# AIGC-Audio/AudioGPT

Hardware: NVIDIA H100
Metric: mel_frames_per_s_vocoded (higher is better)
Workload: dtype f32

## Files before the change

### audiogpt_b200/csrc/tcconv5.cu

```cuda
#include "tapconv.cuh"
#include "tapconv_epi.cuh"
#include "tc_common.cuh"
#include "tc_h16.cuh"
#include "tc_tma.cuh"
#include "models.h"

#include <set>

namespace agpt {

namespace {

constexpr int MAX_NA = 4, MAX_NW = 8;
constexpr int kMaxDyn = 227 * 1024 - 256;
constexpr int kDualDyn = 113 * 1024 - 256;

struct Tc5Smem {
  uint32_t a_hi[MAX_NA], a_lo[MAX_NA], w[MAX_NW], raw[2], rowinfo, rowp, bars, total;
};
__host__ __device__ inline void tc5_layout(Tc5Smem& s, int BN, int MT, int RRA, int NA, int NW, int NR, bool pl = false,
                                           int raw_pitch = 256) {
  uint32_t o = 0;
  for (int i = 0; i < MAX_NA; ++i) { s.a_hi[i] = o; if (i < NA) o += RRA * 128; }
  for (int i = 0; i < MAX_NA; ++i) { s.a_lo[i] = o; if (i < NA) o += RRA * 128; }
// ... 455 lines not shown
        const int a = rowinfo[row];
        const bool ok = (a >= 0) && (ch < P1.Cin);
        const int slot = ((u >> 1) + ((u & 1) << 2)) ^ (((row >> 2) & 1) << 2);
        cp_async16_zfill(dst + row * 128 + (slot << 4), ok ? (ing + a + ch) : P1.in, ok ? 16u : 0u);
      }
      cp_async_commit_();
    };
    if constexpr (HALF) {
      issue_half(0, 0);
      if (NR == 2) issue_half(1, 1);
    } else {
      issue_raw1(0, 0);
      if (NR == 2 && nchunks > 1) issue_raw1(1, 1);
    }
    {
      const int lines = (BN * 4) / 128 > 0 ? (BN * 4) / 128 : 1;
      for (int idx = xt; idx < MT * lines; idx += NWK) {
        const int p = rowp[idx / lines];
        const int co = (idx % lines) * 32;
        if (p >= 0 && co < P2.Cout) {
          asm volatile("prefetch.global.L2 [%0];" ::"l"(P2.res + g * P2.res_gstride + (long)p * P2.res_pitch + co));
          if (P2.epi == EPI_ACC && P2.accumulate)
            asm volatile("prefetch.global.L2 [%0];" ::"l"(P2.out + g * P2.out_gstride + (long)p * P2.out_pitch + co));
        }
      }
    }
    float acc[MB][NJ][NB / 2];
    zero_tile(acc);
    int it = 0, prev = -1;
    auto mma_taps = [&](const TapConvParams& Q, uint32_t ahi0, uint32_t alo0, int ksteps) {
      for (int t = 0; t < Q.ntaps; ++t, ++it) {
        const int s = it % NW;
        mbar_wait(&w_full[s], (uint32_t)((it / NW) & 1));
        const uint32_t shift = (uint32_t)Q.tap_off[t] * 128u;
        mma_group(acc, make_desc(ahi0 + shift), make_desc(alo0 + shift), smem_u32(smem + S.w[s]), ksteps, w_empty, prev);
        prev = s;
      }
    };
    for (int c = 0; c < nchunks; ++c) {
      const int buf = c % NA;
      const int rb = (NR == 2) ? (c & 1) : 0;
      const int kv = min(H_KCH, P1.Cin - c * H_KCH);
      const int nq = ((kv + 15) >> 4) << 1;
      if constexpr (!HALF) {
        if (NR == 2 && c + 1 < nchunks) asm volatile("cp.async.wait_group 1;" ::: "memory");
        else cp_async_wait_all_();
        named_bar_sync(1, NWK);
      }
      uint8_t* ahi = smem + S.a_hi[buf];
      uint8_t* alo = smem + S.a_lo[buf];
      if constexpr (HALF) {
      const int nh = (kv + 31) >> 5;
      for (int h = 0; h < nh; ++h) {
        if (NR == 2 && h + 1 < nh) asm volatile("cp.async.wait_group 1;" ::: "memory");
        else cp_async_wait_all_();
        named_bar_sync(1, NWK);
        const uint8_t* rawb = smem + S.raw[NR == 2 ? h : 0];
#pragma unroll 2
        for (int idx = xt; idx < RRA * 4; idx += NWK) {
          const int row = ((idx >> 5) << 3) + ((idx >> 3) & 3) + (((idx >> 2) & 1) << 2), q = idx & 3, qg = 4 * h + q;
          if (qg >= nq) continue;
          const int sw = ((row >> 2) & 1) << 6;
          const float4 x0 = pro_apply5(P1, *reinterpret_cast<const float4*>(rawb + row * 128 + ((q * 16) ^ sw)), true, nullptr);
          const float4 x1 = pro_apply5(P1, *reinterpret_cast<const float4*>(rawb + row * 128 + ((64 + q * 16) ^ sw)), true, nullptr);
          uint4 hv, lv;
          split8(x0, x1, hv, lv);
          const uint32_t o = sw128(row, qg);
          *reinterpret_cast<uint4*>(ahi + o) = hv;
          *reinterpret_cast<uint4*>(alo + o) = lv;
        }
        if (NR == 1 && h + 1 < nh) {
          named_bar_sync(1, NWK);
          issue_half(h + 1, 0);
        }
      }
      fence_proxy_async();
      named_bar_sync(1, NWK);
      } else {
      const uint8_t* rawb = smem + S.raw[rb];
#pragma unroll 2
      for (int idx = xt; idx < RRA * 8; idx += NWK) {
        const int row = idx >> 3, q = idx & 7;
        if (q >= nq) continue;
        const float4 x0 = pro_apply5(P1, *reinterpret_cast<const float4*>(rawb + row * 256 + q * 16), true, nullptr);
        const float4 x1 = pro_apply5(P1, *reinterpret_cast<const float4*>(rawb + row * 256 + 128 + q * 16), true, nullptr);
        uint4 h, l;
        split8(x0, x1, h, l);
        const uint32_t o = sw128(row, q);
        *reinterpret_cast<uint4*>(ahi + o) = h;
        *reinterpret_cast<uint4*>(alo + o) = l;
      }
      fence_proxy_async();
      named_bar_sync(1, NWK);
      if (c + NR < nchunks) issue_raw1(c + NR, rb);
      }
      mma_taps(P1, smem_u32(ahi) + (uint32_t)(wg * (MT / 2) - lo) * 128u, smem_u32(alo) + (uint32_t)(wg * (MT / 2) - lo) * 128u,
               (kv + 15) >> 4);
      if (NA == 1) {
        mma_drain(acc, w_empty, prev);
        prev = -1;
      }
    }
    mma_drain(acc, w_empty, prev);
    prev = -1;
    named_bar_sync(1, NWK);
    const int nch2 = P2.tc_chunks_h;
    uint8_t* a2 = smem + S.a_hi[0];
    const uint32_t lo_part = (uint32_t)nch2 * P2.R * 128;
    const int r0 = wg * (MT / 2) + (warp & 3) * 16 + (lane >> 2), c0 = 2 * (lane & 3);
    pair_handoff<MT>(acc, P1, P2, a2, nch2, P2.R, Lv, r0, c0, qa, xt, NWK);
    named_bar_sync(1, NWK);
    for (int c = 0; c < nch2; ++c) {
      const uint32_t ahi0 = smem_u32(a2) + (uint32_t)c * P2.R * 128 + (uint32_t)(wg * (MT / 2) - P2.lo_al) * 128u;
      mma_taps(P2, ahi0, ahi0 + lo_part, (min(H_KCH, P2.Cin - c * H_KCH) + 15) >> 4);
    }
    tile_epilogue<BN, MT, HALF ? 1 : 4, false>(acc, P2, g, 0, rowp, smem, S, wg, xt, nullptr);
  } else if (lane == 0) {
    const uint32_t bytes = 2u * BN * 128u;
    const int total2 = P2.tc_chunks_h * P2.ntaps;
    for (int it = 0; it < total + total2; ++it) {
      const uint8_t* src = it < total ? reinterpret_cast<const uint8_t*>(P1.w_h) + (size_t)it * bytes
                                      : reinterpret_cast<const uint8_t*>(P2.w_h) + (size_t)(it - total) * bytes;
      ring_put(smem, S.w, w_full, w_empty, NW, it, src, bytes);
    }
  }
}

template <int BN, int MT>
__global__ void __launch_bounds__(V5_THREADS, 1) tcpair_kernel(const __grid_constant__ TapConvParams P1,
                                                               const __grid_constant__ TapConvParams P2) {
  tcpair_body<BN, MT>(P1, P2);
}
template <int BN>
__global__ void __launch_bounds__(V5_THREADS, 2) tcpair2_kernel(const __grid_constant__ TapConvParams P1,
                                                                const __grid_constant__ TapConvParams P2) {
  tcpair_body<BN, TC_ROWS, true>(P1, P2);
}

constexpr int PIPE_THREADS = 512;
constexpr uint32_t PIPE_STAGE = 2u * 128u * 64u;
__device__ __forceinline__ uint64_t make_desc64(uint32_t saddr) {
  uint64_t d = 0;
  d |= (uint64_t)((saddr & 0x3FFFF) >> 4);
  d |= (uint64_t)1 << 16;
  d |= (uint64_t)(512 >> 4) << 32;
  d |= (uint64_t)2 << 62;
  return d;
}
constexpr int PIPE_MMA = 256, PIPE_DATA = 128;
template <int N> __device__ __forceinline__ void setmaxnreg_inc() { asm volatile("setmaxnreg.inc.sync.aligned.u32 %0;" ::"n"(N)); }
template <int N> __device__ __forceinline__ void setmaxnreg_dec() { asm volatile("setmaxnreg.dec.sync.aligned.u32 %0;" ::"n"(N)); }

constexpr int PIPE_MAX_NW = 8;
struct PipeSmem { uint32_t set[2], w[PIPE_MAX_NW], bars, total; };
__host__ __device__ inline void pipe_layout(PipeSmem& s, int R1, int NW) {
  uint32_t o = 0;
  for (int i = 0; i < 2; ++i) { s.set[i] = o; o += (uint32_t)R1 * 512; }
  for (int i = 0; i < PIPE_MAX_NW; ++i) { s.w[i] = o; if (i < NW) o += PIPE_STAGE; }
  s.bars = o; o += (2 * PIPE_MAX_NW + 4) * 8;
  s.total = o;
}

__global__ void __launch_bounds__(PIPE_THREADS, 1) tcpair_pipe_kernel(const __grid_constant__ TapConvParams P1,
                                                                      const __grid_constant__ TapConvParams P2) {
  constexpr int BN = 128, MT = TC_ROWS;
  extern __shared__ uint8_t smem_raw_[];
  uint8_t* smem = reinterpret_cast<uint8_t*>((reinterpret_cast<uintptr_t>(smem_raw_) + 1023) & ~(uintptr_t)1023);
  const int R1 = P1.R, NW = P1.tc_nw;
  __shared__ PipeSmem S;
  if (threadIdx.x == 0) pipe_layout(S, R1, NW);
  __syncthreads();
  uint64_t* w_full = reinterpret_cast<uint64_t*>(smem + S.bars);
  uint64_t* w_empty = w_full + PIPE_MAX_NW;
  uint64_t* in_full = w_full + 2 * PIPE_MAX_NW;
  uint64_t* acc_full = in_full + 2;

  const int tid = threadIdx.x, warp = tid >> 5, lane = tid & 31;
  const int wg = __shfl_sync(0xffffffffu, tid >> 7, 0);
  int span2 = 0;
  for (int t = 0; t < P2.ntaps; ++t) span2 = max(span2, P2.tap_off[t] - P2.lo_al);
  const int Lv = P1.L, MTO = MT - span2, ntx = (Lv + MTO - 1) / MTO, ntiles = ntx * P1.G;
  const int nloc = (int)blockIdx.x < ntiles ? (ntiles - 1 - (int)blockIdx.x) / (int)gridDim.x + 1 : 0;
  const int lo = P1.lo_al, nch = P1.tc_chunks_h, total1 = 2 * nch * P1.ntaps;
  const int RR2 = P2.R, nch2 = P2.tc_chunks_h, total2 = 2 * nch2 * P2.ntaps;
  auto tile_of = [&](int k, int& g, int& q0) {
    const int T = (int)blockIdx.x + k * (int)gridDim.x;
    g = T / ntx;
    q0 = (T - g * ntx) * MTO;
  };

  if (tid == 0) {
    for (int i = 0; i < NW; ++i) { mbar_init(&w_full[i], 1); mbar_init(&w_empty[i], PIPE_MMA / 32); }
    for (int i = 0; i < 2; ++i) { mbar_init(&in_full[i], PIPE_DATA); mbar_init(&acc_full[i], PIPE_MMA); }
    fence_barrier_init();
  }
  __syncthreads();
  pdl_wait();

  if (wg < 2) {
    setmaxnreg_inc<168>();
    float acc[1][1][BN / 2];
    int it = 0, prev = -1;
    auto mma_taps = [&](const TapConvParams& Q, uint32_t ahi0, uint32_t alo0) {
      for (int t = 0; t < Q.ntaps; ++t)
        for (int hf = 0; hf < 2; ++hf, ++it) {
          const int s = it % NW;
          mbar_wait(&w_full[s], (uint32_t)((it / NW) & 1));
          const uint32_t shift = (uint32_t)Q.tap_off[t] * 128u;
          const uint64_t dah = make_desc(ahi0 + shift) + 4 * hf, dal = make_desc(alo0 + shift) + 4 * hf;
          const uint32_t ws = smem_u32(smem + S.w[s]);
          fence_tile(acc);
          wgmma_fence();
#pragma unroll
          for (int k = 0; k < 2; ++k) {
            const uint64_t ko = (uint64_t)((k * 32) >> 4);
            const uint64_t dwh = make_desc64(ws) + ko, dwl = make_desc64(ws + BN * 64) + ko;
            wgmma_n128(acc[0][0], dah + ko, dwh);
            wgmma_n128(acc[0][0], dal + ko, dwh);
            wgmma_n128(acc[0][0], dah + ko, dwl);
          }
          wgmma_commit();
          wgmma_wait<1>();
          fence_tile(acc);
          if (prev >= 0 && lane == 0) mbar_arrive(&w_empty[prev]);
          prev = s;
        }
    };
    const int r0 = wg * (MT / 2) + (warp & 3) * 16 + (lane >> 2), c0 = 2 * (lane & 3);
    for (int k = 0; k < nloc; ++k) {
      int g, q0;
      tile_of(k, g, q0);
      const int qa = q0 + P2.lo_al;
      uint8_t* set = smem + S.set[k & 1];
      zero_tile(acc);
      mbar_wait(&in_full[k & 1], (uint32_t)((k >> 1) & 1));
      for (int c = 0; c < nch; ++c) {
        const uint32_t ahi0 = smem_u32(set) + (uint32_t)c * R1 * 128 + (uint32_t)(wg * (MT / 2) - lo) * 128u;
        mma_taps(P1, ahi0, ahi0 + (uint32_t)nch * R1 * 128);
      }
      mma_drain(acc, w_empty, prev);
      prev = -1;
      named_bar_sync(1, PIPE_MMA);
      pair_handoff<MT>(acc, P1, P2, set, nch2, RR2, Lv, r0, c0, qa, tid, PIPE_MMA);
      named_bar_sync(1, PIPE_MMA);
      const uint32_t lo_part = (uint32_t)nch2 * RR2 * 128;
      for (int c = 0; c < nch2; ++c) {
        const uint32_t ahi0 = smem_u32(set) + (uint32_t)c * RR2 * 128 + (uint32_t)(wg * (MT / 2) - P2.lo_al) * 128u;
        mma_taps(P2, ahi0, ahi0 + lo_part);
      }
      mma_drain(acc, w_empty, prev);
      prev = -1;
      named_bar_sync(1, PIPE_MMA);
#pragma unroll
      for (int blk = 0; blk < BN / 32; ++blk) stage_block(acc, set + blk * (MT * 128), blk * 32, r0, c0, P2.tc_descale);
      mbar_arrive(&acc_full[k & 1]);
    }
  } else if (wg == 2) {
    setmaxnreg_inc<152>();
    const int dt = tid - PIPE_MMA;
    auto transform = [&](int k) {
      int g, q0;
      tile_of(k, g, q0);
      const int rin = q0 + P2.lo_al + lo;
      const float* __restrict__ ing = P1.in + g * P1.in_gstride;
      uint8_t* set = smem + S.set[k & 1];
      const int items = R1 * nch * 8;
#pragma unroll 4
      for (int idx = dt; idx < items; idx += PIPE_DATA) {
        const int row = idx / (nch * 8), c = (idx >> 3) % nch, q = idx & 7;
        const int r = rin + row, ch = c * H_KCH + 8 * q;
        float4 v0 = make_float4(0.f, 0.f, 0.f, 0.f), v1 = v0;
        if (r >= 0 && r < Lv && ch < P1.Cin) {
          v0 = ldg_stream(ing + (long)r * P1.in_pitch + ch);
          v1 = ldg_stream(ing + (long)r * P1.in_pitch + ch + 4);
        }
        const float4 x0 = pro_apply5(P1, v0, true, nullptr), x1 = pro_apply5(P1, v1, true, nullptr);
        uint4 h, l;
        split8(x0, x1, h, l);
        const uint32_t o = (uint32_t)c * R1 * 128 + sw128(row, q);
        *reinterpret_cast<uint4*>(set + o) = h;
        *reinterpret_cast<uint4*>(set + (uint32_t)nch * R1 * 128 + o) = l;
      }
      fence_proxy_async();
      mbar_arrive(&in_full[k & 1]);
    };
    auto epilogue = [&](int k) {
      int g, q0;
      tile_of(k, g, q0);
      const uint8_t* set = smem + S.set[k & 1];
      const int jc = dt & 7;
      for (int blk = 0; blk < BN / 32; ++blk) {
        const int cb = blk * 32;
        const uint8_t* stg = set + blk * (MT * 128);
        const float4 cv = epi_colvec(P2, g, cb + 4 * jc);
        for (int h = 0; h < 2; ++h) {
          EpiPre pre[4];
          int pp[4];
#pragma unroll
          for (int i = 0; i < 4; ++i) {
            const int row = (dt + (4 * h + i) * PIPE_DATA) >> 3;
            pp[i] = (row < MTO && q0 + row < Lv) ? q0 + row : -1;
            if (pp[i] >= 0) epi_load(P2, g, pp[i], cb + 4 * jc, pre[i]);
          }
#pragma unroll
          for (int i = 0; i < 4; ++i) {
            const int row = (dt + (4 * h + i) * PIPE_DATA) >> 3;
            if (pp[i] >= 0)
              epi_store_cv(P2, g, pp[i], cb + 4 * jc, *reinterpret_cast<const float4*>(stg + sw128(row, jc)), pre[i], cv);
          }
        }
      }
    };
    if (nloc > 0) transform(0);
    for (int k = 0; k < nloc; ++k) {
      if (k + 1 < nloc) transform(k + 1);
      mbar_wait(&acc_full[k & 1], (uint32_t)((k >> 1) & 1));
      epilogue(k);
      named_bar_sync(2, PIPE_DATA);
    }
  } else {
    setmaxnreg_dec<24>();
    if (warp != 12 || lane != 0) return;
    int n_it = 0;
    for (int k = 0; k < nloc; ++k)
      for (int it = 0; it < total1 + total2; ++it, ++n_it) {
        const uint8_t* src = it < total1 ? reinterpret_cast<const uint8_t*>(P1.w_hk) + (size_t)it * PIPE_STAGE
                                         : reinterpret_cast<const uint8_t*>(P2.w_hk) + (size_t)(it - total1) * PIPE_STAGE;
        ring_put(smem, S.w, w_full, w_empty, NW, n_it, src, PIPE_STAGE);
      }
  }
}

constexpr int NARROW_THREADS = 640;
constexpr int NARROW_MMA = 256, NARROW_DATA = 128, NARROW_WG = 128;
constexpr int NARROW_MMA_REGS = 112, NARROW_XF_REGS = 80, NARROW_EPI_REGS = 152;
constexpr int NARROW_MAX_NS = 4, NARROW_MAX_NW = 22;
struct NarrowSmem { uint32_t op[NARROW_MAX_NS], raw[NARROW_MAX_NS], w[NARROW_MAX_NW], bars, total; };
__host__ __device__ inline void narrow_layout(NarrowSmem& s, int BN, int R1, int nbox, int NS, int NW) {
  uint32_t o = 0;
  for (int i = 0; i < NARROW_MAX_NS; ++i) { s.op[i] = o; if (i < NS) o += (uint32_t)R1 * 256; }
  for (int i = 0; i < NARROW_MAX_NS; ++i) { s.raw[i] = o; if (i < NS) o += (uint32_t)R1 * 128 * nbox; }
  for (int i = 0; i < NARROW_MAX_NW; ++i) { s.w[i] = o; if (i < NW) o += 2u * BN * 128; }
  s.bars = o; o += (2 * NARROW_MAX_NW + 4 * NARROW_MAX_NS) * 8;
  s.total = o;
}

template <int BN>
__global__ void __launch_bounds__(NARROW_THREADS, 1) tcpair_narrow_kernel(const __grid_constant__ TapConvParams P1,
                                                                          const __grid_constant__ TapConvParams P2,
                                                                          const __grid_constant__ CUtensorMap tmx) {
  constexpr int NB = tc5_nb(BN), MT = TC_ROWS;
  static_assert(NB == BN && BN <= 64, "narrow pairs: one wgmma column block");
  extern __shared__ uint8_t smem_raw_[];
  uint8_t* smem = reinterpret_cast<uint8_t*>((reinterpret_cast<uintptr_t>(smem_raw_) + 1023) & ~(uintptr_t)1023);
  const int R1 = P1.R, NS = P1.tc_na, NW = P1.tc_nw, nbox = (P1.Cin + 31) >> 5;
  __shared__ NarrowSmem S;
  if (threadIdx.x == 0) narrow_layout(S, BN, R1, nbox, NS, NW);
  __syncthreads();
  uint64_t* w_full = reinterpret_cast<uint64_t*>(smem + S.bars);
  uint64_t* w_empty = w_full + NARROW_MAX_NW;
  uint64_t* raw_full = w_empty + NARROW_MAX_NW;
  uint64_t* in_full = raw_full + NARROW_MAX_NS;
  uint64_t* acc_full = in_full + NARROW_MAX_NS;
  uint64_t* set_free = acc_full + NARROW_MAX_NS;

  const int tid = threadIdx.x, warp = tid >> 5, lane = tid & 31;
  const int wg = __shfl_sync(0xffffffffu, tid >> 7, 0);
  int span2 = 0;
  for (int t = 0; t < P2.ntaps; ++t) span2 = max(span2, P2.tap_off[t] - P2.lo_al);
  const int Lv = P1.L, MTO = MT - span2, ntx = (Lv + MTO - 1) / MTO, ntiles = ntx * P1.G;
  const int nloc = (int)blockIdx.x < ntiles ? (ntiles - 1 - (int)blockIdx.x) / (int)gridDim.x + 1 : 0;
  const int lo = P1.lo_al, RR2 = P2.R;
  const int total1 = P1.ntaps, iters = total1 + P2.ntaps;
  const bool wres = NW == iters;
  auto tile_of = [&](int k, int& g, int& q0) {
    const int T = (int)blockIdx.x + k * (int)gridDim.x;
    g = T / ntx;
    q0 = (T - g * ntx) * MTO;
  };

  if (tid == 0) {
    for (int i = 0; i < NW; ++i) { mbar_init(&w_full[i], 1); mbar_init(&w_empty[i], NARROW_MMA / 32); }
    for (int i = 0; i < NS; ++i) {
      mbar_init(&raw_full[i], 1);
      mbar_init(&in_full[i], NARROW_DATA);
      mbar_init(&acc_full[i], NARROW_WG);
      mbar_init(&set_free[i], NARROW_DATA);
    }
    fence_barrier_init();
  }
  __syncthreads();
  pdl_wait();

  if (wg < 2) {
    setmaxnreg_inc<NARROW_MMA_REGS>();
    float acc[2][1][BN / 2];
    int it = 0, prev = -1;
    auto mma_taps = [&](const TapConvParams& Q, uint32_t ahi0, uint32_t alo0, int ksteps) {
      for (int t = 0; t < Q.ntaps; ++t, ++it) {
        const int s = it % NW;
        mbar_wait(&w_full[s], wres ? 0u : (uint32_t)((it / NW) & 1));
        const uint32_t shift = (uint32_t)Q.tap_off[t] * 128u;
        mma_group(acc, make_desc(ahi0 + shift), make_desc(alo0 + shift), smem_u32(smem + S.w[s]), ksteps,
                  w_empty, wres ? -1 : prev);
        prev = s;
      }
    };
    const int bar = 1 + wg, wt = tid - wg * NARROW_WG;
    const int r0 = (warp & 3) * 16 + (lane >> 2), c0 = 2 * (lane & 3);
    const uint32_t lo_part = (uint32_t)RR2 * 128;
    int k = wg;
    for (; k < nloc; k += 2) {
      int g, q0;
      tile_of(k, g, q0);
      const int qa = q0 + P2.lo_al, s = k % NS;
      uint8_t* set = smem + S.op[s];
      zero_tile(acc);
      mbar_wait(&in_full[s], (uint32_t)((k / NS) & 1));
      {
        const uint32_t ahi0 = smem_u32(set) + (uint32_t)(-lo) * 128u;
        mma_taps(P1, ahi0, ahi0 + (uint32_t)R1 * 128, (P1.Cin + 15) >> 4);
      }
      mma_drain(acc, w_empty, wres ? -1 : prev);
      prev = -1;
      named_bar_sync(bar, NARROW_WG);
      pair_handoff<MT>(acc, P1, P2, set, 1, RR2, Lv, r0, c0, qa, wt, NARROW_WG);
      named_bar_sync(bar, NARROW_WG);
      {
        const uint32_t ahi0 = smem_u32(set) + (uint32_t)(-P2.lo_al) * 128u;
        mma_taps(P2, ahi0, ahi0 + lo_part, (P2.Cin + 15) >> 4);
      }
      mma_drain(acc, w_empty, wres ? -1 : prev);
      prev = -1;
      named_bar_sync(bar, NARROW_WG);
#pragma unroll
      for (int blk = 0; blk < BN / 32; ++blk) stage_block(acc, set + blk * (MT * 128), blk * 32, r0, c0, P2.tc_descale);
      mbar_arrive(&acc_full[s]);
    }
    if (!wres && k < 2 * ((nloc + 1) / 2))
      for (int t = 0; t < iters; ++t, ++it) {
        const int s = it % NW;
        mbar_wait(&w_full[s], (uint32_t)((it / NW) & 1));
        if (lane == 0) mbar_arrive(&w_empty[s]);
      }
  } else if (wg == 2) {
    setmaxnreg_dec<NARROW_XF_REGS>();
    const int dt = tid - NARROW_MMA;
    const int lq = P1.Cin > 32 ? 3 : (P1.Cin > 16 ? 2 : 1);
    for (int k = 0; k < nloc; ++k) {
      const int s = k % NS;
      mbar_wait(&raw_full[s], (uint32_t)((k / NS) & 1));
      const uint8_t* raw = smem + S.raw[s];
      uint8_t* set = smem + S.op[s];
#pragma unroll 2
      for (int idx = dt; idx < (R1 << lq); idx += NARROW_DATA) {
        const int row = idx >> lq, q = idx & ((1 << lq) - 1);
        const uint8_t* rr = raw + (uint32_t)(q >> 2) * R1 * 128 + row * 128;
        const int j0 = (2 * q) & 7, sw = row & 7;
        const float4 x0 = pro_apply5(P1, *reinterpret_cast<const float4*>(rr + ((j0 ^ sw) << 4)), true, nullptr);
        const float4 x1 = pro_apply5(P1, *reinterpret_cast<const float4*>(rr + (((j0 + 1) ^ sw) << 4)), true, nullptr);
        uint4 h, l;
        split8(x0, x1, h, l);
        const uint32_t o = sw128(row, q);
        *reinterpret_cast<uint4*>(set + o) = h;
        *reinterpret_cast<uint4*>(set + (uint32_t)R1 * 128 + o) = l;
      }
      fence_proxy_async();
      mbar_arrive(&in_full[s]);
    }
  } else if (wg == 3) {
    setmaxnreg_inc<NARROW_EPI_REGS>();
// ... 409 lines not shown
  smem = (size_t)S.total + 1024;
  return smem <= (size_t)kMaxDyn;
}

static bool tcpair_plan_dual(TapConvParams& P, int BN, long a_min, int iters, size_t& smem) {
  if (P.tc_chunks_h != 1) return false;
  const long abytes = 2L * P.R * 128, wbytes = 2L * BN * 128;
  const int NA = (int)cdiv(std::max(a_min, 2L * TC_ROWS * 128), abytes);
  if (NA > MAX_NA) return false;
  for (int NR = cdiv(P.Cin, 32); NR >= 1; --NR) {
    Tc5Smem S;
    tc5_layout(S, BN, TC_ROWS, P.R, NA, 2, NR, false, 128);
    const long spare = (long)kDualDyn - 1024 - S.total;
    if (spare < 0) continue;
    const int NW = (int)std::min<long>(std::min<long>(MAX_NW, std::max(2, iters)), 2 + spare / wbytes);
    tc5_layout(S, BN, TC_ROWS, P.R, NA, NW, NR, false, 128);
    P.tc_bn = BN; P.tc_na = NA; P.tc_nw = NW; P.tc_nr = NR;
    smem = (size_t)S.total + 1024;
    return smem <= (size_t)kDualDyn;
  }
  return false;
}

static void tc_func_attrs(const void* kern, bool dual) {
  int dev = 0;
  AGPT_CUDA(cudaGetDevice(&dev));
  static std::set<std::pair<const void*, int>> done;
  if (done.count({kern, dev})) return;
  AGPT_CUDA(cudaFuncSetAttribute(kern, cudaFuncAttributeMaxDynamicSharedMemorySize, dual ? kDualDyn : kMaxDyn));
  if (dual) AGPT_CUDA(cudaFuncSetAttribute(kern, cudaFuncAttributePreferredSharedMemoryCarveout, cudaSharedmemCarveoutMaxShared));
  done.insert({kern, dev});
}
template <typename... KArgs, typename... Args>
static void tc_launch(void (*kern)(KArgs...), bool dual, dim3 grid, dim3 block, size_t smem, cudaStream_t st, Args&&... args) {
  tc_func_attrs(reinterpret_cast<const void*>(kern), dual);
  launch_pdl(kern, grid, block, smem, st, std::forward<Args>(args)...);
}

static auto tcconv5_kern(int BN, int MT) {
  if (MT == TC_TALL) return BN == 64 ? tcconv5_kernel<64, TC_TALL> : tcconv5_kernel<32, TC_TALL>;
  return BN == 128 ? tcconv5_kernel<128, TC_ROWS>
                   : BN == 96 ? tcconv5_kernel<96, TC_ROWS> : BN == 64 ? tcconv5_kernel<64, TC_ROWS> : tcconv5_kernel<32, TC_ROWS>;
}
static auto tcconv5_pl_kern(int BN, int MT) {
  if (MT == TC_TALL) return BN == 64 ? tcconv5_pl_kernel<64, TC_TALL> : tcconv5_pl_kernel<32, TC_TALL>;
  return BN == 128 ? tcconv5_pl_kernel<128, TC_ROWS>
                   : BN == 96 ? tcconv5_pl_kernel<96, TC_ROWS>
                              : BN == 64 ? tcconv5_pl_kernel<64, TC_ROWS> : tcconv5_pl_kernel<32, TC_ROWS>;
}
static auto tcpair_kern(int BN, int MT) {
  if (MT == TC_TALL) return BN == 64 ? tcpair_kernel<64, TC_TALL> : tcpair_kernel<32, TC_TALL>;
  return BN == 128 ? tcpair_kernel<128, TC_ROWS> : BN == 64 ? tcpair_kernel<64, TC_ROWS> : tcpair_kernel<32, TC_ROWS>;
}

static int tc5_sms() {
  int dev = 0;
  AGPT_CUDA(cudaGetDevice(&dev));
  static int sms_dev[64] = {0};
  if (!sms_dev[dev & 63]) AGPT_CUDA(cudaDeviceGetAttribute(&sms_dev[dev & 63], cudaDevAttrMultiProcessorCount, dev));
  return sms_dev[dev & 63];
}

static bool tc5_tall(const TapConvParams& P, int bn, long tall_tiles, int sms) {
  return P.tc_tall && bn <= 64 && !P.Wreal && !P.strips && tall_tiles >= 4L * sms;
}

struct PlMaps { CUtensorMap hi, lo; };
static PlMaps pl_tensor_maps(const TapConvParams& P) {
  AGPT_CHECK(!P.Wreal && !P.strips, "plane-fed tap-GEMMs run over plain 1-D rows");
  PlMaps m;
  const int br = pl_box_rows(P.R);
  AGPT_CHECK(tma_encode_rows_h(&m.hi, P.pi_hi, P.Cin, P.L, P.G, P.in_pitch, P.in_gstride, br) &&
                 tma_encode_rows_h(&m.lo, P.pi_lo, P.Cin, P.L, P.G, P.in_pitch, P.in_gstride, br),
             "cannot encode the operand-plane tensor maps");
  return m;
}

static bool tcconv5_try(TapConvParams P, int BN, int MT, cudaStream_t st) {
  tc5_rows(P, MT);
  size_t smem = 0;
  if (!tc5_plan(P, BN, MT, 0, P.tc_chunks_h * P.ntaps, smem)) return false;
  const int Lv = tc_lv(P);
  dim3 grid(cdiv(Lv, MT), cdiv(P.Cout, BN), tc_groups(P));
  tapconv_note_launch(1, BN, MT, P.pi_hi ? 1 : 0);
  if (P.pi_hi) {
    const PlMaps m = pl_tensor_maps(P);
    tc_launch(tcconv5_pl_kern(BN, MT), false, grid, dim3(V5_THREADS), smem, st, P, m.hi, m.lo);
  } else {
    tc_launch(tcconv5_kern(BN, MT), false, grid, dim3(V5_THREADS), smem, st, P);
  }
  if (MT == TC_TALL) profile_count_tall();
  if (P.pi_hi) profile_count_plane();
  return true;
}

HTile pick_h_tile(const TapConvParams& P, int sms) {
  const int Lv = tc_lv(P);
  const long rt = (long)cdiv(Lv, TC_ROWS) * tc_groups(P);
  static int allow96 = -1;
  if (allow96 < 0) { const char* e = getenv("AGPT_TC_BN96"); allow96 = (e && e[0] == '0') ? 0 : 1; }
  auto cost = [](int bn) { return bn == 128 ? 1.0 : (bn == 96 ? 0.82 : (bn == 64 ? 0.62 : 0.45)); };
  HTile best{P.tc_bn, P.w_h, rt * cdiv(P.Cout, P.tc_bn), TC_ROWS};
  double bs = (double)cdiv(best.ntiles, (long)sms) * cost(P.tc_bn);
  auto consider = [&](int bn, const float* w) {
    if (!w) return;
    const long nt = rt * cdiv(P.Cout, bn);
    const double sc = (double)cdiv(nt, (long)sms) * cost(bn);
    if (sc < bs - 1e-9) { bs = sc; best = HTile{bn, w, nt, TC_ROWS}; }
  };
  if (P.tc_bn == 128) consider(64, P.w_h64);
  if (P.tc_bn == 128 && allow96) consider(96, P.w_h96);
  const long tall = (long)cdiv(Lv, TC_TALL) * tc_groups(P) * cdiv(P.Cout, best.bn);
  if (tc5_tall(P, best.bn, tall, sms)) { best.mt = TC_TALL; best.ntiles = tall; }
  return best;
}

static bool tcpair_try(TapConvParams P1, TapConvParams P2, int MT, bool dual, cudaStream_t st) {
  const int BN = P1.tc_bn;
  tc5_rows(P1, MT);
  const int span2 = tc5_rows(P2, MT);
  P2.tc_bn = BN;
  size_t smem = 0;
  const long a2bytes = 2L * P2.tc_chunks_h * P2.R * 128;
  const int iters = P1.tc_chunks_h * P1.ntaps + P2.tc_chunks_h * P2.ntaps;
  if (dual ? !tcpair_plan_dual(P1, BN, a2bytes, iters, smem) : !tc5_plan(P1, BN, MT, a2bytes, iters, smem)) return false;
  dim3 grid(cdiv(tc_lv(P1), MT - span2), 1, tc_groups(P1));
  const auto dual_kern = BN == 64 ? tcpair2_kernel<64> : tcpair2_kernel<32>;
  if (dual) {
    tc_func_attrs(reinterpret_cast<const void*>(dual_kern), true);
    int per_sm = 0;
    AGPT_CUDA(cudaOccupancyMaxActiveBlocksPerMultiprocessor(&per_sm, dual_kern, V5_THREADS, smem));
    if (per_sm != 2) return false;
  }
  void* rec = profile_begin_pair(P1, P2, st);
  tapconv_note_launch(1, BN, MT, 0);
  if (dual) {
    tc_launch(dual_kern, true, grid, dim3(V5_THREADS), smem, st, P1, P2);
    profile_count_dual();
  } else {
    tc_launch(tcpair_kern(BN, MT), false, grid, dim3(V5_THREADS), smem, st, P1, P2);
    if (MT == TC_TALL) profile_count_tall();
  }
  profile_end(rec, st);
  count_launch(1);
  AGPT_CUDA(cudaGetLastError());
  return true;
}

static bool tcpair_pipe_try(TapConvParams P1, TapConvParams P2, cudaStream_t st) {
  if (!P1.tc_pipe || P1.tc_bn != 128 || P1.Cin != 128 || P1.Cout != 128 || P2.Cout != 128 || !P1.w_hk || !P2.w_hk)
    return false;
  tc5_rows(P1, TC_ROWS);
  const int span2 = tc5_rows(P2, TC_ROWS);
  if (P2.R > P1.R) return false;
  const long wbytes = PIPE_STAGE;
  PipeSmem S;
  pipe_layout(S, P1.R, 0);
  const long spare = (long)kMaxDyn - 1024 - (long)S.total;
  if (spare < 4 * wbytes) return false;
  const int iters = 2 * (P1.tc_chunks_h * P1.ntaps + P2.tc_chunks_h * P2.ntaps);
  P1.tc_nw = (int)std::min<long>(std::min<long>(PIPE_MAX_NW, iters), spare / wbytes);
  P2.tc_bn = 128;
  pipe_layout(S, P1.R, P1.tc_nw);
  const size_t smem = (size_t)S.total + 1024;
  const long tiles = (long)cdiv(P1.L, TC_ROWS - span2) * P1.G;
  dim3 grid((unsigned)std::min<long>(tiles, tc5_sms()));
  void* rec = profile_begin_pair(P1, P2, st);
  tapconv_note_launch(1, 128, TC_ROWS, 0);
  tc_launch(tcpair_pipe_kernel, false, grid, dim3(PIPE_THREADS), smem, st, P1, P2);
  profile_count_pipe();
  profile_end(rec, st);
  count_launch(1);
  AGPT_CUDA(cudaGetLastError());
  return true;
}

static bool tcpair_dual(const TapConvParams& P1) {
  return P1.tc_dual && P1.tc_bn <= 64;
}

static bool tcpair_narrow_try(TapConvParams P1, TapConvParams P2, cudaStream_t st) {
  const int BN = P1.tc_bn, iters = P1.ntaps + P2.ntaps;
  if (!P1.tc_narrow_pipe || (BN != 64 && BN != 32) || (BN == 64 && iters > 14) || P1.Cin > BN ||
      P2.res != P1.in || P2.res_pitch != P1.in_pitch || P2.res_gstride != P1.in_gstride)
    return false;
  const int span1 = tc5_rows(P1, TC_ROWS);
  const int span2 = tc5_rows(P2, TC_ROWS);
  if (P2.R > P1.R || P1.R > 256 || P1.lo_al > 0 || P2.lo_al > 0 || (P1.lo_al + span1) + (P2.lo_al + span2) < 0)
    return false;
  const int nbox = cdiv(P1.Cin, 32);
  const long wbytes = 2L * BN * 128, set = 256L * P1.R + 128L * nbox * P1.R;
  NarrowSmem S;
  narrow_layout(S, BN, P1.R, nbox, 0, 0);
  const long avail = (long)kMaxDyn - 1024 - (long)S.total;
  int NS = 2, NW;
  if (avail - iters * wbytes >= 2 * set) {
    NW = iters;
    NS = (int)std::min<long>(NARROW_MAX_NS, (avail - iters * wbytes) / set);
  } else {
    NW = (int)std::min<long>(iters, (avail - NS * set) / wbytes);
    if (NW < 2) return false;
  }
  CUtensorMap tmx;
  if (!tma_encode_rows(&tmx, P1.in, P1.Cin, P1.L, P1.G, P1.in_pitch, P1.in_gstride, P1.R)) return false;
  P1.tc_na = NS; P1.tc_nw = NW;
  P2.tc_bn = BN;
  narrow_layout(S, BN, P1.R, nbox, NS, NW);
  const size_t smem = (size_t)S.total + 1024;
  const long tiles = (long)cdiv(P1.L, TC_ROWS - span2) * P1.G;
  dim3 grid((unsigned)std::min<long>(tiles, tc5_sms()));
  void* rec = profile_begin_pair(P1, P2, st);
  tapconv_note_launch(1, BN, TC_ROWS, 0);
  tc_launch(BN == 64 ? tcpair_narrow_kernel<64> : tcpair_narrow_kernel<32>, false, grid, dim3(NARROW_THREADS), smem, st, P1,
            P2, tmx);
  profile_count_dual();
  profile_count_narrow_pipe();
  profile_end(rec, st);
  count_launch(1);
  AGPT_CUDA(cudaGetLastError());
  return true;
}

bool tcpair_launch(TapConvParams P1, TapConvParams P2, cudaStream_t st) {
  if (!tcconv_supported(P1) || !P2.w_h) return false;
  const int BN = P1.tc_bn;
  if (P1.pi_hi || P2.po_hi) return false;
  if (P2.tc_bn != BN || P1.Cout > BN || P2.Cin != P1.Cout || P2.Cout > BN || P1.Wreal || P2.Wreal || P1.strips ||
      P1.G != P2.G || P1.L != P2.L || P1.pro != PRO_LRELU || P2.pro != PRO_LRELU || (P2.epi != EPI_RES && P2.epi != EPI_ACC))
    return false;
  if (tcpair_pipe_try(P1, P2, st)) return true;
  if (tcpair_dual(P1) && (tcpair_narrow_try(P1, P2, st) || tcpair_try(P1, P2, TC_ROWS, true, st))) return true;
  const int span2 = tc5_rows(P2, TC_TALL);
  if (tc5_tall(P1, BN, (long)cdiv(tc_lv(P1), TC_TALL - span2) * tc_groups(P1), tc5_sms()) &&
      tcpair_try(P1, P2, TC_TALL, false, st))
    return true;
  return tcpair_try(P1, P2, TC_ROWS, false, st);
}

static bool tcconv_pipe_try(TapConvParams P, const HTile& c, cudaStream_t st) {
  if (!P.tc_conv_pipe || !P.pi_hi || P.Wreal || P.strips || c.bn != 128 || c.mt != TC_ROWS ||
      (P.epi != EPI_BIAS && P.epi != EPI_RES && P.epi != EPI_ACC))
    return false;
  P.w_h = c.w;
  P.tc_bn = 128;
  tc5_rows(P, TC_ROWS);
  const int PR = pl_rows(P.R);
  const long abytes = 256L * PR, wbytes = 2L * 128 * 128;
  CpipeSmem S;
  cpipe_layout(S, PR, 0, 0);
  const long avail = (long)kMaxDyn - 1024 - (long)S.total;
  int NA = std::min(MAX_NA, std::max(2, P.tc_chunks_h));
  while (NA > 2 && NA * abytes + 3 * wbytes > avail) --NA;
  const int NW = (int)std::min<long>(MAX_NW, (avail - NA * abytes) / wbytes);
  if (NW < 2) return false;
  P.tc_na = NA; P.tc_nw = NW;
  cpipe_layout(S, PR, NA, NW);
  const size_t smem = (size_t)S.total + 1024;
  const int units = cdiv(P.L, TC_ROWS) * P.G * cdiv(P.Cout, 128);
  const PlMaps m = pl_tensor_maps(P);
  tapconv_note_launch(1, 128, TC_ROWS, 1);
  tc_launch(tcconv_pipe_pl_kernel, false, dim3(cpipe_grid(units, tc5_sms())), dim3(CPIPE_THREADS), smem, st, P, m.hi, m.lo);
  profile_count_plane();
  profile_count_conv_pipe();
  return true;
}

bool tcconv5_launch(TapConvParams P, cudaStream_t st) {
  if (!P.w_h) return false;
  const HTile c = pick_h_tile(P, tc5_sms());
  if (tcconv_pipe_try(P, c, st)) return true;
  if (c.bn != P.tc_bn || c.mt != TC_ROWS) {
    TapConvParams Q = P;
    Q.w_h = c.w;
    if (tcconv5_try(Q, c.bn, c.mt, st)) return true;
  }
  return tcconv5_try(P, P.tc_bn, TC_ROWS, st);
}

}
```

Before: 208,800.

## Add single-stage split-buffer mode to pipelined tcpair kernel for larger layers

Adds a single-stage mode to the pipelined paired tap-conv kernel. It applies when the second layer's input rows exceed the first's or double-buffered shared memory would not fit. In that mode the input buffer and the handoff/epilogue buffer are separate regions, guarded by new in_empty and acc_empty mbarriers. This lets the next tile's transform overlap the current tile's second conv, and lets more layer pairs use the warp-specialized pipe path instead of falling back. The cost is weaker overlap than double buffering and extra barrier waits.

```diff
diff --git a/audiogpt_b200/csrc/tcconv5.cu b/audiogpt_b200/csrc/tcconv5.cu
--- a/audiogpt_b200/csrc/tcconv5.cu
+++ b/audiogpt_b200/csrc/tcconv5.cu
@@ -631,12 +631,13 @@
 template <int N> __device__ __forceinline__ void setmaxnreg_dec() { asm volatile("setmaxnreg.dec.sync.aligned.u32 %0;" ::"n"(N)); }
 
 constexpr int PIPE_MAX_NW = 8;
-struct PipeSmem { uint32_t set[2], w[PIPE_MAX_NW], bars, total; };
-__host__ __device__ inline void pipe_layout(PipeSmem& s, int R1, int NW) {
+struct PipeSmem { uint32_t x[2], y[2], w[PIPE_MAX_NW], bars, total; };
+__host__ __device__ inline void pipe_layout(PipeSmem& s, int R1, int RR2, int NS, int NW) {
   uint32_t o = 0;
-  for (int i = 0; i < 2; ++i) { s.set[i] = o; o += (uint32_t)R1 * 512; }
+  for (int i = 0; i < NS; ++i) { s.x[i] = s.y[i] = o; o += (uint32_t)R1 * 512; }
+  if (NS == 1) { s.y[0] = o; o += RR2 * 512 > 65536 ? (uint32_t)RR2 * 512 : 65536u; }
   for (int i = 0; i < PIPE_MAX_NW; ++i) { s.w[i] = o; if (i < NW) o += PIPE_STAGE; }
-  s.bars = o; o += (2 * PIPE_MAX_NW + 4) * 8;
+  s.bars = o; o += (2 * PIPE_MAX_NW + 8) * 8;
   s.total = o;
 }
 
@@ -645,14 +646,16 @@
   constexpr int BN = 128, MT = TC_ROWS;
   extern __shared__ uint8_t smem_raw_[];
   uint8_t* smem = reinterpret_cast<uint8_t*>((reinterpret_cast<uintptr_t>(smem_raw_) + 1023) & ~(uintptr_t)1023);
-  const int R1 = P1.R, NW = P1.tc_nw;
+  const int R1 = P1.R, NW = P1.tc_nw, NS = P1.tc_na, sh = NS - 1;
   __shared__ PipeSmem S;
-  if (threadIdx.x == 0) pipe_layout(S, R1, NW);
+  if (threadIdx.x == 0) pipe_layout(S, R1, P2.R, NS, NW);
   __syncthreads();
   uint64_t* w_full = reinterpret_cast<uint64_t*>(smem + S.bars);
   uint64_t* w_empty = w_full + PIPE_MAX_NW;
   uint64_t* in_full = w_full + 2 * PIPE_MAX_NW;
-  uint64_t* acc_full = in_full + 2;
+  uint64_t* in_empty = in_full + 2;
+  uint64_t* acc_full = in_full + 4;
+  uint64_t* acc_empty = in_full + 6;
 
   const int tid = threadIdx.x, warp = tid >> 5, lane = tid & 31;
   const int wg = __shfl_sync(0xffffffffu, tid >> 7, 0);
@@ -670,7 +673,12 @@
 
   if (tid == 0) {
     for (int i = 0; i < NW; ++i) { mbar_init(&w_full[i], 1); mbar_init(&w_empty[i], PIPE_MMA / 32); }
-    for (int i = 0; i < 2; ++i) { mbar_init(&in_full[i], PIPE_DATA); mbar_init(&acc_full[i], PIPE_MMA); }
+    for (int i = 0; i < NS; ++i) {
+      mbar_init(&in_full[i], PIPE_DATA);
+      mbar_init(&in_empty[i], 1);
+      mbar_init(&acc_full[i], PIPE_MMA);
+      mbar_init(&acc_empty[i], 1);
+    }
     fence_barrier_init();
   }
   __syncthreads();
@@ -709,30 +717,36 @@
     for (int k = 0; k < nloc; ++k) {
       int g, q0;
       tile_of(k, g, q0);
-      const int qa = q0 + P2.lo_al;
-      uint8_t* set = smem + S.set[k & 1];
+      const int qa = q0 + P2.lo_al, s = k & sh;
+      const uint32_t ph = (uint32_t)(k >> sh) & 1;
+      uint8_t* xs = smem + S.x[s];
+      uint8_t* ys = smem + S.y[s];
       zero_tile(acc);
-      mbar_wait(&in_full[k & 1], (uint32_t)((k >> 1) & 1));
+      mbar_wait(&in_full[s], ph);
       for (int c = 0; c < nch; ++c) {
-        const uint32_t ahi0 = smem_u32(set) + (uint32_t)c * R1 * 128 + (uint32_t)(wg * (MT / 2) - lo) * 128u;
+        const uint32_t ahi0 = smem_u32(xs) + (uint32_t)c * R1 * 128 + (uint32_t)(wg * (MT / 2) - lo) * 128u;
         mma_taps(P1, ahi0, ahi0 + (uint32_t)nch * R1 * 128);
       }
       mma_drain(acc, w_empty, prev);
       prev = -1;
       named_bar_sync(1, PIPE_MMA);
-      pair_handoff<MT>(acc, P1, P2, set, nch2, RR2, Lv, r0, c0, qa, tid, PIPE_MMA);
+      if (NS == 1) {
+        if (tid == 0) mbar_arrive(&in_empty[0]);
+        if (k >= 1) mbar_wait(&acc_empty[0], ph ^ 1u);
+      }
+      pair_handoff<MT>(acc, P1, P2, ys, nch2, RR2, Lv, r0, c0, qa, tid, PIPE_MMA);
       named_bar_sync(1, PIPE_MMA);
       const uint32_t lo_part = (uint32_t)nch2 * RR2 * 128;
       for (int c = 0; c < nch2; ++c) {
-        const uint32_t ahi0 = smem_u32(set) + (uint32_t)c * RR2 * 128 + (uint32_t)(wg * (MT / 2) - P2.lo_al) * 128u;
+        const uint32_t ahi0 = smem_u32(ys) + (uint32_t)c * RR2 * 128 + (uint32_t)(wg * (MT / 2) - P2.lo_al) * 128u;
         mma_taps(P2, ahi0, ahi0 + lo_part);
       }
       mma_drain(acc, w_empty, prev);
       prev = -1;
       named_bar_sync(1, PIPE_MMA);
 #pragma unroll
-      for (int blk = 0; blk < BN / 32; ++blk) stage_block(acc, set + blk * (MT * 128), blk * 32, r0, c0, P2.tc_descale);
-      mbar_arrive(&acc_full[k & 1]);
+      for (int blk = 0; blk < BN / 32; ++blk) stage_block(acc, ys + blk * (MT * 128), blk * 32, r0, c0, P2.tc_descale);
+      mbar_arrive(&acc_full[s]);
     }
   } else if (wg == 2) {
     setmaxnreg_inc<152>();
@@ -742,7 +756,8 @@
       tile_of(k, g, q0);
       const int rin = q0 + P2.lo_al + lo;
       const float* __restrict__ ing = P1.in + g * P1.in_gstride;
-      uint8_t* set = smem + S.set[k & 1];
+      uint8_t* set = smem + S.x[k & sh];
+      if (NS == 1 && k >= 1) mbar_wait(&in_empty[0], (uint32_t)(k & 1) ^ 1u);
       const int items = R1 * nch * 8;
 #pragma unroll 4
       for (int idx = dt; idx < items; idx += PIPE_DATA) {
@@ -761,12 +776,12 @@
         *reinterpret_cast<uint4*>(set + (uint32_t)nch * R1 * 128 + o) = l;
       }
       fence_proxy_async();
-      mbar_arrive(&in_full[k & 1]);
+      mbar_arrive(&in_full[k & sh]);
     };
     auto epilogue = [&](int k) {
       int g, q0;
       tile_of(k, g, q0);
-      const uint8_t* set = smem + S.set[k & 1];
+      const uint8_t* set = smem + S.y[k & sh];
       const int jc = dt & 7;
       for (int blk = 0; blk < BN / 32; ++blk) {
         const int cb = blk * 32;
@@ -793,9 +808,10 @@
     if (nloc > 0) transform(0);
     for (int k = 0; k < nloc; ++k) {
       if (k + 1 < nloc) transform(k + 1);
-      mbar_wait(&acc_full[k & 1], (uint32_t)((k >> 1) & 1));
+      mbar_wait(&acc_full[k & sh], (uint32_t)((k >> sh) & 1));
       epilogue(k);
       named_bar_sync(2, PIPE_DATA);
+      if (NS == 1 && dt == 0) mbar_arrive(&acc_empty[0]);
     }
   } else {
     setmaxnreg_dec<24>();
@@ -1511,16 +1527,22 @@
     return false;
   tc5_rows(P1, TC_ROWS);
   const int span2 = tc5_rows(P2, TC_ROWS);
-  if (P2.R > P1.R) return false;
   const long wbytes = PIPE_STAGE;
   PipeSmem S;
-  pipe_layout(S, P1.R, 0);
-  const long spare = (long)kMaxDyn - 1024 - (long)S.total;
-  if (spare < 4 * wbytes) return false;
+  auto spare = [&](int NS) {
+    pipe_layout(S, P1.R, P2.R, NS, 0);
+    return (long)kMaxDyn - 1024 - (long)S.total;
+  };
+  int NS = 2;
+  if (P2.R > P1.R || spare(2) < 4 * wbytes) {
+    NS = 1;
+    if (spare(1) < 3 * wbytes) return false;
+  }
   const int iters = 2 * (P1.tc_chunks_h * P1.ntaps + P2.tc_chunks_h * P2.ntaps);
-  P1.tc_nw = (int)std::min<long>(std::min<long>(PIPE_MAX_NW, iters), spare / wbytes);
+  P1.tc_na = NS;
+  P1.tc_nw = (int)std::min<long>(std::min<long>(PIPE_MAX_NW, iters), spare(NS) / wbytes);
   P2.tc_bn = 128;
-  pipe_layout(S, P1.R, P1.tc_nw);
+  pipe_layout(S, P1.R, P2.R, NS, P1.tc_nw);
   const size_t smem = (size_t)S.total + 1024;
   const long tiles = (long)cdiv(P1.L, TC_ROWS - span2) * P1.G;
   dim3 grid((unsigned)std::min<long>(tiles, tc5_sms()));
```

Result: faster. 213,700 (median of 6 runs) (+2.4%).

## Add single-input-set A/B buffer mode to pipelined pair conv kernel

Applied to the files above, without the earlier changes.

Templates the pipelined pair-conv kernel on the number of shared-memory staging sets and adds a mode with one input set plus a separate output set, coordinated by new a_free/b_free mbarriers. The host picks this mode when the second conv needs more rows than the first, or when double buffering leaves too little space for the weight ring. It lowers the ring minimum from four to three stages. Layers that previously fell back to a slower non-pipelined path can now use the warp-specialized pipeline, at the cost of less overlap between input transform and MMA.

```diff
diff --git a/audiogpt_b200/csrc/tcconv5.cu b/audiogpt_b200/csrc/tcconv5.cu
--- a/audiogpt_b200/csrc/tcconv5.cu
+++ b/audiogpt_b200/csrc/tcconv5.cu
@@ -632,27 +632,34 @@
 
 constexpr int PIPE_MAX_NW = 8;
 struct PipeSmem { uint32_t set[2], w[PIPE_MAX_NW], bars, total; };
-__host__ __device__ inline void pipe_layout(PipeSmem& s, int R1, int NW) {
+__host__ __device__ inline void pipe_layout(PipeSmem& s, int R1, int R2, int nset, int NW) {
   uint32_t o = 0;
-  for (int i = 0; i < 2; ++i) { s.set[i] = o; o += (uint32_t)R1 * 512; }
+  s.set[0] = o; o += (uint32_t)R1 * 512;
+  s.set[1] = o; o += (uint32_t)(nset == 2 ? R1 : R2) * 512;
   for (int i = 0; i < PIPE_MAX_NW; ++i) { s.w[i] = o; if (i < NW) o += PIPE_STAGE; }
-  s.bars = o; o += (2 * PIPE_MAX_NW + 4) * 8;
+  s.bars = o; o += (2 * PIPE_MAX_NW + 6) * 8;
   s.total = o;
 }
 
+template <int NSET>
 __global__ void __launch_bounds__(PIPE_THREADS, 1) tcpair_pipe_kernel(const __grid_constant__ TapConvParams P1,
                                                                       const __grid_constant__ TapConvParams P2) {
-  constexpr int BN = 128, MT = TC_ROWS;
+  constexpr int BN = 128, MT = TC_ROWS, nset = NSET;
+  constexpr bool ab = NSET == 1;
   extern __shared__ uint8_t smem_raw_[];
   uint8_t* smem = reinterpret_cast<uint8_t*>((reinterpret_cast<uintptr_t>(smem_raw_) + 1023) & ~(uintptr_t)1023);
   const int R1 = P1.R, NW = P1.tc_nw;
   __shared__ PipeSmem S;
-  if (threadIdx.x == 0) pipe_layout(S, R1, NW);
+  if (threadIdx.x == 0) pipe_layout(S, R1, P2.R, nset, NW);
   __syncthreads();
   uint64_t* w_full = reinterpret_cast<uint64_t*>(smem + S.bars);
   uint64_t* w_empty = w_full + PIPE_MAX_NW;
   uint64_t* in_full = w_full + 2 * PIPE_MAX_NW;
   uint64_t* acc_full = in_full + 2;
+  uint64_t* a_free = acc_full + 2;
+  uint64_t* b_free = a_free + 1;
+  auto in_set = [&](int k) { return smem + S.set[k % nset]; };
+  auto out_set = [&](int k) { return smem + S.set[ab ? 1 : (k & 1)]; };
 
   const int tid = threadIdx.x, warp = tid >> 5, lane = tid & 31;
   const int wg = __shfl_sync(0xffffffffu, tid >> 7, 0);
@@ -671,6 +678,8 @@
   if (tid == 0) {
     for (int i = 0; i < NW; ++i) { mbar_init(&w_full[i], 1); mbar_init(&w_empty[i], PIPE_MMA / 32); }
     for (int i = 0; i < 2; ++i) { mbar_init(&in_full[i], PIPE_DATA); mbar_init(&acc_full[i], PIPE_MMA); }
+    mbar_init(a_free, PIPE_MMA);
+    mbar_init(b_free, PIPE_DATA);
     fence_barrier_init();
   }
   __syncthreads();
@@ -710,16 +719,19 @@
       int g, q0;
       tile_of(k, g, q0);
       const int qa = q0 + P2.lo_al;
-      uint8_t* set = smem + S.set[k & 1];
+      uint8_t* ins = in_set(k);
+      uint8_t* set = out_set(k);
       zero_tile(acc);
-      mbar_wait(&in_full[k & 1], (uint32_t)((k >> 1) & 1));
+      mbar_wait(&in_full[k % nset], (uint32_t)((k / nset) & 1));
       for (int c = 0; c < nch; ++c) {
-        const uint32_t ahi0 = smem_u32(set) + (uint32_t)c * R1 * 128 + (uint32_t)(wg * (MT / 2) - lo) * 128u;
+        const uint32_t ahi0 = smem_u32(ins) + (uint32_t)c * R1 * 128 + (uint32_t)(wg * (MT / 2) - lo) * 128u;
         mma_taps(P1, ahi0, ahi0 + (uint32_t)nch * R1 * 128);
       }
       mma_drain(acc, w_empty, prev);
       prev = -1;
+      if (ab) mbar_arrive(a_free);
       named_bar_sync(1, PIPE_MMA);
+      if (ab && k > 0) mbar_wait(b_free, (uint32_t)((k - 1) & 1));
       pair_handoff<MT>(acc, P1, P2, set, nch2, RR2, Lv, r0, c0, qa, tid, PIPE_MMA);
       named_bar_sync(1, PIPE_MMA);
       const uint32_t lo_part = (uint32_t)nch2 * RR2 * 128;
@@ -732,7 +744,7 @@
       named_bar_sync(1, PIPE_MMA);
 #pragma unroll
       for (int blk = 0; blk < BN / 32; ++blk) stage_block(acc, set + blk * (MT * 128), blk * 32, r0, c0, P2.tc_descale);
-      mbar_arrive(&acc_full[k & 1]);
+      mbar_arrive(&acc_full[k % nset]);
     }
   } else if (wg == 2) {
     setmaxnreg_inc<152>();
@@ -742,7 +754,7 @@
       tile_of(k, g, q0);
       const int rin = q0 + P2.lo_al + lo;
       const float* __restrict__ ing = P1.in + g * P1.in_gstride;
-      uint8_t* set = smem + S.set[k & 1];
+      uint8_t* set = in_set(k);
       const int items = R1 * nch * 8;
 #pragma unroll 4
       for (int idx = dt; idx < items; idx += PIPE_DATA) {
@@ -761,12 +773,12 @@
         *reinterpret_cast<uint4*>(set + (uint32_t)nch * R1 * 128 + o) = l;
       }
       fence_proxy_async();
-      mbar_arrive(&in_full[k & 1]);
+      mbar_arrive(&in_full[k % nset]);
     };
     auto epilogue = [&](int k) {
       int g, q0;
       tile_of(k, g, q0);
-      const uint8_t* set = smem + S.set[k & 1];
+      const uint8_t* set = out_set(k);
       const int jc = dt & 7;
       for (int blk = 0; blk < BN / 32; ++blk) {
         const int cb = blk * 32;
@@ -792,10 +804,14 @@
     };
     if (nloc > 0) transform(0);
     for (int k = 0; k < nloc; ++k) {
-      if (k + 1 < nloc) transform(k + 1);
-      mbar_wait(&acc_full[k & 1], (uint32_t)((k >> 1) & 1));
+      if (k + 1 < nloc) {
+        if (ab) mbar_wait(a_free, (uint32_t)(k & 1));
+        transform(k + 1);
+      }
+      mbar_wait(&acc_full[k % nset], (uint32_t)((k / nset) & 1));
       epilogue(k);
-      named_bar_sync(2, PIPE_DATA);
+      if (ab) mbar_arrive(b_free);
+      else named_bar_sync(2, PIPE_DATA);
     }
   } else {
     setmaxnreg_dec<24>();
@@ -1511,22 +1527,27 @@
     return false;
   tc5_rows(P1, TC_ROWS);
   const int span2 = tc5_rows(P2, TC_ROWS);
-  if (P2.R > P1.R) return false;
   const long wbytes = PIPE_STAGE;
   PipeSmem S;
-  pipe_layout(S, P1.R, 0);
-  const long spare = (long)kMaxDyn - 1024 - (long)S.total;
-  if (spare < 4 * wbytes) return false;
+  int nset = 2;
+  pipe_layout(S, P1.R, P2.R, nset, 0);
+  long spare = (long)kMaxDyn - 1024 - (long)S.total;
+  if (P2.R > P1.R || spare < 4 * wbytes) {
+    nset = 1;
+    pipe_layout(S, P1.R, P2.R, nset, 0);
+    spare = (long)kMaxDyn - 1024 - (long)S.total;
+    if (spare < 3 * wbytes) return false;
+  }
   const int iters = 2 * (P1.tc_chunks_h * P1.ntaps + P2.tc_chunks_h * P2.ntaps);
   P1.tc_nw = (int)std::min<long>(std::min<long>(PIPE_MAX_NW, iters), spare / wbytes);
   P2.tc_bn = 128;
-  pipe_layout(S, P1.R, P1.tc_nw);
+  pipe_layout(S, P1.R, P2.R, nset, P1.tc_nw);
   const size_t smem = (size_t)S.total + 1024;
   const long tiles = (long)cdiv(P1.L, TC_ROWS - span2) * P1.G;
   dim3 grid((unsigned)std::min<long>(tiles, tc5_sms()));
   void* rec = profile_begin_pair(P1, P2, st);
   tapconv_note_launch(1, 128, TC_ROWS, 0);
-  tc_launch(tcpair_pipe_kernel, false, grid, dim3(PIPE_THREADS), smem, st, P1, P2);
+  tc_launch(nset == 2 ? tcpair_pipe_kernel<2> : tcpair_pipe_kernel<1>, false, grid, dim3(PIPE_THREADS), smem, st, P1, P2);
   profile_count_pipe();
   profile_end(rec, st);
   count_launch(1);
```

Result: faster. 208,600 before, 213,900 after, median of 6 (+2.6%).
